# Fabstir/fabstir-vectordb

Hardware: AMD Instinct MI355X
Metric: k-NN queries/sec at recall@10>=0.95, 1Mx384 f32 (higher is better)
Workload: dtype f32

## Files before the change

fabstir-vectordb_amd/csrc/fvdb_hip.cpp:

```cpp
#include "fvdb_internal.h"

#include <unistd.h>

#include <algorithm>
#include <atomic>
#include <cmath>
#include <condition_variable>
#include <mutex>
#include <cstdio>
#include <cstdlib>
#include <cstring>
#include <map>
#include <new>
#include <string>
#include <vector>

#include "common.h"
#include "pool.h"
#include "kernels_misc.h"
#include "kernels_scan.h"
#include "kernels_wide.h"
#include "kernels_range.h"
#include "kernels_rank.h"
#include "kernels_curve.h"
#include "kernels_coarse.h"
#include "kernels_mfma.h"
#include "kernels_mfma_wg.h"
#include "kernels_util.h"
#include "kernels_maint.h"
#include "kernels_rows.h"

using namespace fvdb;


enum FbWord : uint32_t {
  FB_COARSE = 0,
  FB_SCAN = 1,
  FB_REASONS = 2,
  FB_OVERFLOW = 2,
  FB_REFINED = 6,
  FB_WORDS = 8,
};
constexpr size_t kFbBytes = FB_WORDS * 4;
constexpr size_t kFbAllBytes = 2 * kFbBytes;
constexpr uint32_t kFbReasonWords = 5;

enum StageEvent {
  EV_COARSE_BEGIN = 0,
  EV_COARSE_SCANNED,
  EV_COARSE_DONE,
  EV_SCAN_BEGIN,
  EV_SCAN_DONE,
  EV_FINE_DONE,
  EV_FILTER_BEGIN,
  EV_FILTER_DONE,
  EV_COUNT
};

enum ScalWord : uint32_t {
  SC_COARSE_ITEMS = 0,
  SC_COARSE_HEAD = 1,
  SC_FINE_ITEMS = 2,
  SC_FINE_HEAD = 3,
  SC_STATS = 4,
};
constexpr size_t kScalarsBytes = 64;

struct IvfScratch {
  std::mutex enq;
  bool pend_filter = false;
  bool pending_profile = false, pend_coarse = false, pend_fine = false, collecting = false;
  DBuf s_qnorm, s_A;
  DBuf s_qh, s_qn2, s_thr, s_tA, s_pa, s_surv, s_scnt, s_fail, s_mslots;
  DBuf s_sdist, s_probes2;
  DBuf s_q, s_cpart, s_probes, s_cnt, s_fill, s_eoff, s_ioff, s_entries;
  DBuf s_part, s_scalars, s_ceoff, s_cioff;
  DBuf s_wbase, s_arena;
  DBuf s_wgbase;
  DBuf s_gwords, s_group;
  DBuf s_rbase, s_rarena;
  DBuf s_qual;
  DBuf s_clive, s_cprobes, s_ckeys, s_cval;
  DBuf s_in, s_slots, s_ids, s_clusters, s_out_ids, s_out_dist, s_out_cnt, s_cdist;
  DBuf s_fslots, s_frows;
  DevEvent fetch_done;
  DevEvent sev[EV_COUNT];
  uint32_t* scalar(ScalWord w) const { return s_scalars.as<uint32_t>() + w; }
};

struct fvdb_ivf : IvfScratch {
  static constexpr uint32_t kSlots = 16;
  IvfScratch spare[kSlots - 1];
  static constexpr uint32_t kLeases = 8;
  IvfScratch lease_set[kLeases];
  fvdb_ctx* lease_ctx[kLeases] = {};
  uint32_t lease_busy = 0;
  std::mutex mu;
  std::condition_variable lease_cv;
  std::atomic<IvfScratch*> last_set{nullptr};
  std::atomic<fvdb_ctx*> last_ctx{nullptr};
  fvdb_ctx* ctx = nullptr;
  uint32_t d = 0, dpad = 0, d4 = 0, nlist = 0;
  bool trained = false;
  bool f16 = false;

  std::vector<float> h_centroids;
  DBuf d_centroids_rm;
  DBuf d_cent_pad;
  DBuf d_cnorm, d_cnmax;
  DBuf s_fallbacks;
  uint32_t* fb_word(FbWord w, bool masked = false) const { return s_fallbacks.as<uint32_t>() + (masked ? FB_WORDS : 0) + w; }
  int coarse_mode = 0;
  int scan_mode = 0;
  HBuf h_fb;
  uint64_t mfma_q = 0;
  uint64_t fb_seen = 0, q_seen = 0;
  uint32_t exact_batches_left = 0;
  uint32_t backoff_len = 0;
  uint64_t overflow_seen = 0, overflow_q = 0;
  uint32_t refine_batches_left = 0;
  DBuf d_mfma_stamps;
  int mfma_stamps_launch = 0;
  DBuf d_xmax;
  Pool cpool;
  DBuf c_off, c_blocks, c_glob;

  Pool pool;
  std::vector<std::vector<uint32_t>> list_blocks;
  std::vector<uint32_t> list_len;
  uint64_t total_rows = 0;
  uint64_t mutations = 0;
  uint32_t max_list_blocks = 0;
  bool table_dirty = true;
  DBuf t_off, t_blocks, t_glob, t_len;
  std::vector<uint32_t> glob_blocks_host;
  bool glob_set = false;

  DBuf m_seq, m_dest, m_ids;
  fvdb_ivf* m_src = nullptr;
  uint64_t m_rows = 0;
  bool m_assigned = false;
  bool m_store_job = false;
  fvdb_maintenance_info_t m_info{};

  fvdb_search_stats last_stats{};
  float stage_ms[8] = {0, 0, 0, 0, 0, 0, 0, 0};
  uint64_t stage_calls = 0;
};

namespace {
struct Env {
  fvdb_ctx* ctx;
  IvfScratch* S;
  const uint64_t* live = nullptr;
};
inline IvfScratch& slot_scratch(fvdb_ivf* ivf, uint32_t slot) { return slot == 0 ? *ivf : ivf->spare[slot - 1]; }
inline const uint64_t* live_words(const fvdb_ivf* ivf, const Env& E) { return E.live ? E.live : ivf->pool.valid(); }
inline PoolView list_pool(const fvdb_ivf* ivf, const Env& E) {
  PoolView v = ivf->pool.view();
  v.valid = live_words(ivf, E);
  return v;
}
}


namespace {

struct IvfKnobs {
  static int num(const char* name, int unset) { return getenv(name) ? atoi(getenv(name)) : unset; }
  static bool has(const char* name) { return getenv(name) != nullptr; }
  static int tiles(int m) { return m >= 4 ? 4 : (m >= 2 ? 2 : 1); }
  bool coarse_exact = has("FVDB_COARSE_EXACT");
  bool scan_exact = has("FVDB_SCAN_EXACT");
  uint32_t scan_wgs_per_cu = (uint32_t)num("FVDB_SCAN_WGS_PER_CU", 8);
  int segb = num("FVDB_SEGB", 0);
  bool no_shared_thr = has("FVDB_NO_SHARED_THR");
  int mfma_m = tiles(num("FVDB_MFMA_M", 2));
  int mfma_segb = num("FVDB_MFMA_SEGB", 0);
  uint32_t mfma_wgs_per_cu = (uint32_t)std::max(1, num("FVDB_MFMA_WGS_PER_CU", 2));
  bool mfma_groups_in_item = num("FVDB_MFMA_GROUPS_IN_ITEM", 0) != 0;
  bool mfma_wg = num("FVDB_MFMA_WG", 1) != 0;
  int mfma_wg_m = num("FVDB_MFMA_WG_M", 4) >= 4 ? 4 : 2;
  uint32_t mfma_wg_segb = (uint32_t)std::max(4, num("FVDB_MFMA_WG_SEGB", 16));
  uint32_t mfma_wg_per_cu = (uint32_t)std::max(1, num("FVDB_MFMA_WG_PER_CU", 2));
  int mfma_wg_tail_pct = num("FVDB_MFMA_WG_TAIL_PCT", 25);
  int mfma_wg_segb_tail = num("FVDB_MFMA_WG_SEGB_TAIL", 4);
  uint32_t mfma_cap_a = (uint32_t)std::max(1, num("FVDB_MFMA_CAP_A", 4));
  bool mfma_threshold_pass = has("FVDB_MFMA_THRESHOLD_PASS");
  uint32_t mfma_segb_a = (uint32_t)std::max(1, num("FVDB_MFMA_SEGB_A", 1));
  bool mfma_no_refine = has("FVDB_MFMA_NO_REFINE");
#ifdef FVDB_MFMA_STAMPS_BUILD
  int mfma_stamps = num("FVDB_MFMA_STAMPS", 0);
#endif
};
const IvfKnobs& ivf_knobs() {
  static const IvfKnobs knobs{};
  return knobs;
}

struct ScanLaunch {
  PoolView pool;
  const uint32_t* list_off;
  const uint32_t* list_blocks;
  uint32_t nlist;
  const uint32_t* entry_off;
  const uint32_t* item_off;
  const uint2* entries;
  const uint32_t* n_items;
  uint32_t* head;
  const float* queries;
  uint32_t dpad, segb, k, nprobe, maxsegs;
  uint2* part;
  uint32_t max_items = 0;
  bool f16 = false;
};

inline int kr_for(uint32_t k) { return k <= 64 ? 1 : (k <= 128 ? 2 : 4); }
inline uint32_t q_for(uint32_t k) { return k <= 64 ? 16u : (k <= 128 ? 8u : 4u); }

template <int Q, int KR, int ROLE, int ST>
void launch_scan_t(fvdb_ctx* ctx, const ScanLaunch& s) {
  uint32_t grid = (uint32_t)ctx->num_cus * ivf_knobs().scan_wgs_per_cu;
  if (s.max_items) grid = std::min(grid, std::max<uint32_t>(1u, (s.max_items + 3) / 4));
  hipLaunchKernelGGL((scan_topk_kernel<Q, KR, ROLE, ST>), dim3(grid), dim3(256), 0, ctx->stream, s.pool.data, s.pool.valid,
                     s.pool.d4, s.list_off, s.list_blocks, s.nlist, s.entry_off, s.item_off, (const u32x2*)s.entries,
                     s.n_items, s.head, s.queries, s.dpad, s.segb, s.k, s.nprobe, s.maxsegs, (u32x2*)s.part);
}

template <int ROLE, int ST>
void launch_scan_rs(fvdb_ctx* ctx, const ScanLaunch& s) {
  switch (kr_for(s.k)) {
    case 1: launch_scan_t<16, 1, ROLE, ST>(ctx, s); break;
    case 2: launch_scan_t<8, 2, ROLE, ST>(ctx, s); break;
    default: launch_scan_t<4, 4, ROLE, ST>(ctx, s); break;
  }
}
template <int ROLE>
void launch_scan_r(fvdb_ctx* ctx, const ScanLaunch& s) {
  if (s.f16) launch_scan_rs<ROLE, 1>(ctx, s); else launch_scan_rs<ROLE, 0>(ctx, s);
}
enum { ROLE_COARSE = 0, ROLE_LIST = 1, ROLE_ALL = 2 };
void launch_scan(fvdb_ctx* ctx, const ScanLaunch& s, int role) {
  if (role == ROLE_COARSE) launch_scan_r<ROLE_COARSE>(ctx, s);
  else if (role == ROLE_LIST) launch_scan_r<ROLE_LIST>(ctx, s);
  else launch_scan_r<ROLE_ALL>(ctx, s);
}

void launch_merge(fvdb_ctx* ctx, const MergeArgs& m) {
  const uint32_t grid = cdiv(m.B, 4);
  switch (kr_for(m.k)) {
    case 1: hipLaunchKernelGGL((merge_topk_kernel<1>), dim3(grid), dim3(256), 0, ctx->stream, m); break;
    case 2: hipLaunchKernelGGL((merge_topk_kernel<2>), dim3(grid), dim3(256), 0, ctx->stream, m); break;
    default: hipLaunchKernelGGL((merge_topk_kernel<4>), dim3(grid), dim3(256), 0, ctx->stream, m); break;
  }
}

int upload_table(fvdb_ivf* ivf) {
  fvdb_ctx* ctx = ivf->ctx;
  std::lock_guard<std::mutex> lk(ivf->mu);
  if (!ivf->table_dirty) return FVDB_OK;
  std::vector<uint32_t> off(ivf->nlist + 1, 0), blocks;
  std::vector<uint32_t> glob(ivf->nlist, 0);
  uint32_t mx = 0;
  for (uint32_t L = 0; L < ivf->nlist; ++L) {
    off[L] = (uint32_t)blocks.size();
    blocks.insert(blocks.end(), ivf->list_blocks[L].begin(), ivf->list_blocks[L].end());
    mx = std::max<uint32_t>(mx, (uint32_t)ivf->list_blocks[L].size());
    glob[L] = ivf->glob_set ? ivf->glob_blocks_host[L] : (uint32_t)ivf->list_blocks[L].size();
  }
  off[ivf->nlist] = (uint32_t)blocks.size();
  ivf->max_list_blocks = mx;
  HIPCHK(ctx, ivf->t_off.ensure(off.size() * 4));
  HIPCHK(ctx, ivf->t_blocks.ensure(std::max<size_t>(blocks.size(), 1) * 4));
  HIPCHK(ctx, ivf->t_glob.ensure(glob.size() * 4));
  HIPCHK(ctx, hipMemcpyAsync(ivf->t_off.p, off.data(), off.size() * 4, hipMemcpyHostToDevice, ctx->stream));
  if (!blocks.empty())
    HIPCHK(ctx, hipMemcpyAsync(ivf->t_blocks.p, blocks.data(), blocks.size() * 4, hipMemcpyHostToDevice, ctx->stream));
  HIPCHK(ctx, hipMemcpyAsync(ivf->t_glob.p, glob.data(), glob.size() * 4, hipMemcpyHostToDevice, ctx->stream));
  HIPCHK(ctx, ivf->t_len.ensure((size_t)ivf->nlist * 4));
  HIPCHK(ctx, hipMemcpyAsync(ivf->t_len.p, ivf->list_len.data(), (size_t)ivf->nlist * 4, hipMemcpyHostToDevice,
                             ctx->stream));
  HIPCHK(ctx, hipStreamSynchronize(ctx->stream));
  ivf->table_dirty = false;
  return FVDB_OK;
}

int padded_queries(fvdb_ivf* ivf, const Env& E, const float* q_dev, uint32_t B, const float** out) {
  fvdb_ctx* ctx = E.ctx;
  IvfScratch& S = *E.S;
  if (ivf->d == ivf->dpad) {
    *out = q_dev;
    return FVDB_OK;
  }
  HIPCHK(ctx, S.s_q.ensure((size_t)B * ivf->dpad * 4));
  const uint64_t tot = (uint64_t)B * ivf->dpad;
  hipLaunchKernelGGL(pad_rows_kernel, dim3(cdiv(tot, 256)), dim3(256), 0, ctx->stream, q_dev, ivf->d, ivf->dpad,
                     (uint64_t)B, S.s_q.as<float>());
  *out = S.s_q.as<float>();
  return FVDB_OK;
}

inline void mark(const fvdb_ivf* ivf, const Env& E, StageEvent e) {
  if (ivf->ctx->profiling) (void)hipEventRecord(E.S->sev[e], E.ctx->stream);
}

struct Batch {
  const float* qpad;
  const uint32_t* probes;
  uint32_t B, k, np;
  uint64_t* out_ids;
  float* out_dist;
  uint32_t* out_counts;
  uint64_t* out_keys;
  const float* given_thr = nullptr;
  bool glob_keys = false;
  const uint64_t* const* words = nullptr;
  const uint32_t* group = nullptr;
  const float* radius = nullptr;
  uint32_t* out_totals = nullptr;
};

inline ListTable list_table(const fvdb_ivf* ivf) {
  return ListTable{ivf->t_off.as<uint32_t>(), ivf->t_blocks.as<uint32_t>(), ivf->nlist};
}

MergeArgs merge_args(const PoolView& pool, const ListTable& lists, const uint32_t* glob_blocks, const DBuf& part,
                     uint32_t maxsegs, uint32_t segb, const Batch& b) {
  MergeArgs m{};
  m.pool = pool;
  m.lists = lists;
  m.probes = b.probes;
  m.glob_blocks = glob_blocks;
  m.part = part.as<uint2>();
  m.B = b.B;
  m.k = b.k;
  m.nprobe = b.np;
  m.maxsegs = maxsegs;
  m.segb = segb;
  m.out_ids = b.out_ids;
  m.out_dist = b.out_dist;
  m.out_counts = b.out_counts;
  m.out_keys = b.out_keys;
  return m;
}

constexpr uint64_t kRankArenaBytes = 256ull << 20;
int check_rank(fvdb_ctx* ctx, const fvdb_ivf* ivf, uint32_t np) {
  if (np > FVDB_MAX_K && ivf->nlist > kRankSortMaxLists)
    FAIL(ctx, FVDB_E_UNSUPPORTED, "nprobe above FVDB_MAX_K needs an index of at most 16384 lists");
  return FVDB_OK;
}

int run_coarse_rank(fvdb_ivf* ivf, const Env& E, const float* qpad, uint32_t B, uint32_t kc, uint32_t* out_probes,
                    float* out_dist) {
  fvdb_ctx* ctx = E.ctx;
  IvfScratch& S = *E.S;
  int rc = check_rank(ctx, ivf, kc);
  if (rc) return rc;
  const uint32_t cblocks = ivf->cpool.used_blocks, n = cblocks * 64;
  uint32_t P = 1;
  while (P < n) P <<= 1;
  const uint32_t lds = P * 8;
  const uint32_t threads = std::min<uint32_t>(kRankThreads, std::max<uint32_t>(64, P / 2));
  const uint32_t chunk = (uint32_t)std::min<uint64_t>(B, std::max<uint64_t>(1, kRankArenaBytes / ((uint64_t)n * 4)));
  HIPCHK(ctx, S.s_rarena.ensure((size_t)chunk * n * 4));
  HIPCHK(ctx, S.s_rbase.ensure((size_t)chunk * 2 * 4));
  HIPCHK(ctx, S.s_entries.ensure((size_t)chunk * 8));
  HIPCHK(ctx, S.s_ceoff.ensure(16));
  HIPCHK(ctx, S.s_cioff.ensure(16));
  HIPCHK(ctx, S.s_scalars.ensure(kScalarsBytes));
  HIPCHK(ctx, hipFuncSetAttribute((const void*)rank_sort_kernel, hipFuncAttributeMaxDynamicSharedMemorySize,
                                  (int)(kRankSortMaxLists * 8)));
  const ListTable clist{ivf->c_off.as<uint32_t>(), ivf->c_blocks.as<uint32_t>(), 1};
  const PoolView cpool = ivf->cpool.view();
  const uint32_t grid = (uint32_t)ctx->num_cus * ivf_knobs().scan_wgs_per_cu;
  mark(ivf, E, EV_COARSE_BEGIN);
  for (uint32_t o = 0; o < B; o += chunk) {
    const uint32_t b = std::min(chunk, B - o);
    hipLaunchKernelGGL(plan_all_kernel, dim3(cdiv(b, 256)), dim3(256), 0, ctx->stream, b, cblocks, 1u, 16u,
                       S.s_ceoff.as<uint32_t>(), S.s_cioff.as<uint32_t>(), S.s_entries.as<uint2>(),
                       S.scalar(SC_COARSE_ITEMS), S.scalar(SC_COARSE_HEAD));
    hipLaunchKernelGGL(rank_base_kernel, dim3(cdiv(b, 256)), dim3(256), 0, ctx->stream, b, cblocks, S.s_rbase.as<uint32_t>());
    const uint32_t items = cblocks * cdiv(b, 16);
    hipLaunchKernelGGL(wide_score_kernel<0>, dim3(std::min(grid, std::max<uint32_t>(1u, cdiv(items, 4)))), dim3(256), 0,
                       ctx->stream, cpool.data, cpool.valid, cpool.d4, clist.off, clist.blocks, 1u, S.s_ceoff.as<uint32_t>(),
                       S.s_cioff.as<uint32_t>(), (const u32x2*)S.s_entries.as<uint2>(), S.scalar(SC_COARSE_ITEMS),
                       S.scalar(SC_COARSE_HEAD), qpad + (size_t)o * ivf->dpad, ivf->dpad, 1u, 1u, S.s_rbase.as<uint32_t>(),
                       S.s_rarena.as<uint32_t>(), (uint64_t)n);
    if (o + b == B) mark(ivf, E, EV_COARSE_SCANNED);
    RankArgs r{};
    r.pool = cpool;
    r.lists = clist;
    r.arena = S.s_rarena.as<uint32_t>();
    r.n = n;
    r.P = P;
    r.np = kc;
    r.out_probes = out_probes + (size_t)o * kc;
    r.out_dist = out_dist ? out_dist + (size_t)o * kc : nullptr;
    hipLaunchKernelGGL(rank_sort_kernel, dim3(b), dim3(threads), lds, ctx->stream, r);
  }
  mark(ivf, E, EV_COARSE_DONE);
  HIPCHK(ctx, hipGetLastError());
  return FVDB_OK;
}

int run_coarse(fvdb_ivf* ivf, const Env& E, const float* qpad, uint32_t B, uint32_t kc, uint32_t* out_probes,
               float* out_dist) {
  fvdb_ctx* ctx = E.ctx;
  IvfScratch& S = *E.S;
  if (kc > FVDB_MAX_K) return run_coarse_rank(ivf, E, qpad, B, kc, out_probes, out_dist);
  if (ivf->coarse_mode == 0 && !ivf_knobs().coarse_exact && ivf->dpad % 16 == 0 && kc <= 48 && ivf->nlist >= 64 && B > 0 &&
      (uint64_t)B * ivf->nlist < (1ull << 31)) {
    const uint32_t nlist = ivf->nlist;
    const float* cpad = ivf->d == ivf->dpad ? ivf->d_centroids_rm.as<float>() : ivf->d_cent_pad.as<float>();
    HIPCHK(ctx, S.s_qnorm.ensure((size_t)B * 4));
    HIPCHK(ctx, S.s_A.ensure((size_t)B * nlist * 4));
    mark(ivf, E, EV_COARSE_BEGIN);
    hipLaunchKernelGGL(row_sqnorm_wave_kernel, dim3(cdiv(B, 4)), dim3(256), 0, ctx->stream, qpad, ivf->dpad, ivf->dpad, B,
                       S.s_qnorm.as<float>());
    const uint32_t waves = cdiv(B, 32) * cdiv(nlist, 64);
    hipLaunchKernelGGL(coarse_gemm_kernel, dim3(cdiv(waves, 4)), dim3(256), 0, ctx->stream, qpad, cpad,
                       S.s_qnorm.as<float>(), ivf->d_cnorm.as<float>(), B, nlist, ivf->dpad, S.s_A.as<float>());
    mark(ivf, E, EV_COARSE_SCANNED);
    hipLaunchKernelGGL(coarse_select_kernel, dim3(cdiv(B, 4)), dim3(256), 0, ctx->stream, S.s_A.as<float>(), qpad, cpad,
                       S.s_qnorm.as<float>(), ivf->d_cnmax.as<float>(), B, nlist, ivf->d, ivf->dpad, 64u, kc,
                       out_probes, out_dist, ivf->fb_word(FB_COARSE));
    mark(ivf, E, EV_COARSE_DONE);
    HIPCHK(ctx, hipGetLastError());
    return FVDB_OK;
  }
  const uint32_t cblocks = ivf->cpool.used_blocks;
  const uint32_t segb = 1, Q = q_for(kc);
  const uint32_t maxsegs = cblocks;
  HIPCHK(ctx, S.s_cpart.ensure((size_t)B * maxsegs * kc * 8));
  HIPCHK(ctx, S.s_entries.ensure((size_t)B * std::max<uint32_t>(kc, 1) * 8));
  HIPCHK(ctx, S.s_ceoff.ensure(16));
  HIPCHK(ctx, S.s_cioff.ensure(16));
  HIPCHK(ctx, S.s_scalars.ensure(kScalarsBytes));
  hipLaunchKernelGGL(plan_all_kernel, dim3(cdiv(std::max<uint32_t>(B, 1), 256)), dim3(256), 0, ctx->stream, B, cblocks,
                     segb, Q, S.s_ceoff.as<uint32_t>(), S.s_cioff.as<uint32_t>(), S.s_entries.as<uint2>(),
                     S.scalar(SC_COARSE_ITEMS), S.scalar(SC_COARSE_HEAD));
  const ListTable clist{ivf->c_off.as<uint32_t>(), ivf->c_blocks.as<uint32_t>(), 1};
  ScanLaunch s{ivf->cpool.view(), clist.off, clist.blocks, 1, S.s_ceoff.as<uint32_t>(), S.s_cioff.as<uint32_t>(),
               S.s_entries.as<uint2>(), S.scalar(SC_COARSE_ITEMS), S.scalar(SC_COARSE_HEAD), qpad, ivf->dpad, segb, kc, 1,
               maxsegs, S.s_cpart.as<uint2>(), cdiv(cblocks, segb) * cdiv(B, Q)};
  mark(ivf, E, EV_COARSE_BEGIN);
  launch_scan(ctx, s, ROLE_COARSE);
  mark(ivf, E, EV_COARSE_SCANNED);
  MergeArgs m = merge_args(ivf->cpool.view(), clist, ivf->c_glob.as<uint32_t>(), S.s_cpart, maxsegs, segb,
                           Batch{qpad, nullptr, B, kc, 1, nullptr, out_dist, nullptr, nullptr});
  m.out_probes = out_probes;
  launch_merge(ctx, m);
  mark(ivf, E, EV_COARSE_DONE);
  HIPCHK(ctx, hipGetLastError());
  return FVDB_OK;
}

uint32_t segb_for(uint32_t max_blocks, uint32_t B, uint32_t nprobe) {
  const uint64_t pairs = (uint64_t)B * nprobe;
  if (max_blocks >= 4096) return 16;
  if (pairs >= 4096) return 4;
  if (pairs >= 512) return 2;
  return 1;
}
uint32_t pick_segb(fvdb_ivf* ivf, uint32_t B, uint32_t nprobe) {
  const int forced = ivf_knobs().segb;
  return forced > 0 ? (uint32_t)forced : segb_for(ivf->max_list_blocks, B, nprobe);
}
uint64_t queries_per_gib(uint32_t max_blocks, uint32_t segb, uint32_t k, uint32_t np) {
  const uint64_t per_q = (uint64_t)np * std::max<uint32_t>(1, cdiv(max_blocks, segb)) * k * 8;
  return (1ull << 30) / std::max<uint64_t>(per_q, 1);
}

void launch_plan(fvdb_ivf* ivf, const Env& E, const uint32_t* probes, uint32_t n, uint32_t np, uint32_t segb, uint32_t Q,
                 unsigned long long* stats, uint32_t* rezero_cnt, uint32_t lsplit = 0xFFFFFFFFu, uint32_t segb_tail = 0) {
  fvdb_ctx* ctx = E.ctx;
  IvfScratch& S = *E.S;
  const uint32_t* list_off = ivf->t_off.as<uint32_t>();
  hipLaunchKernelGGL(plan_count_kernel, dim3(cdiv(n, 256)), dim3(256), 0, ctx->stream, probes, n, S.s_cnt.as<uint32_t>(),
                     list_off);
  hipLaunchKernelGGL(plan_scan_kernel, dim3(1), dim3(1024), 0, ctx->stream, S.s_cnt.as<uint32_t>(), list_off,
                     ivf->t_len.as<uint32_t>(), ivf->nlist, segb, Q, S.s_eoff.as<uint32_t>(), S.s_ioff.as<uint32_t>(),
                     S.s_fill.as<uint32_t>(), S.scalar(SC_FINE_ITEMS), S.scalar(SC_FINE_HEAD), stats, rezero_cnt, lsplit,
                     segb_tail);
  hipLaunchKernelGGL(plan_fill_kernel, dim3(cdiv(n, 256)), dim3(256), 0, ctx->stream, probes, n, np,
                     S.s_eoff.as<uint32_t>(), S.s_fill.as<uint32_t>(), S.s_entries.as<uint2>(), list_off);
}
inline unsigned long long* scan_stats(const IvfScratch& S) { return (unsigned long long*)S.scalar(SC_STATS); }

int plan_scratch(fvdb_ivf* ivf, const Env& E, uint32_t B, uint32_t np) {
  fvdb_ctx* ctx = E.ctx;
  IvfScratch& S = *E.S;
  const uint32_t nlist = ivf->nlist;
  HIPCHK(ctx, S.s_cnt.ensure((size_t)nlist * 4));
  HIPCHK(ctx, S.s_fill.ensure((size_t)nlist * 4));
  HIPCHK(ctx, S.s_eoff.ensure((size_t)(nlist + 1) * 4));
  HIPCHK(ctx, S.s_ioff.ensure((size_t)(nlist + 1) * 4));
  HIPCHK(ctx, S.s_entries.ensure((size_t)B * np * 8));
  return FVDB_OK;
}

int run_fine_exact(fvdb_ivf* ivf, const Env& E, const Batch& b, int role) {
  fvdb_ctx* ctx = E.ctx;
  IvfScratch& S = *E.S;
  const uint32_t nlist = ivf->nlist;
  const uint32_t segb = pick_segb(ivf, b.B, b.np), Q = q_for(b.k);
  const uint32_t maxsegs = std::max<uint32_t>(1, cdiv(ivf->max_list_blocks, segb));
  const uint64_t part_elems = (uint64_t)b.B * b.np * maxsegs * b.k;
  if (part_elems >= (1ull << 32)) FAIL(ctx, FVDB_E_UNSUPPORTED, "batch too large for one launch (sub-batch it)");
  int rc = plan_scratch(ivf, E, b.B, b.np);
  if (rc) return rc;
  HIPCHK(ctx, S.s_part.ensure((size_t)part_elems * 8));
  HIPCHK(ctx, S.s_scalars.ensure(kScalarsBytes));
  HIPCHK(ctx, hipMemsetAsync(S.s_cnt.p, 0, (size_t)nlist * 4, ctx->stream));
  launch_plan(ivf, E, b.probes, b.B * b.np, b.np, segb, Q, scan_stats(S), nullptr);
  mark(ivf, E, EV_SCAN_BEGIN);
  const ListTable lists = list_table(ivf);
  ScanLaunch s{list_pool(ivf, E), lists.off, lists.blocks, nlist, S.s_eoff.as<uint32_t>(), S.s_ioff.as<uint32_t>(),
               S.s_entries.as<uint2>(), S.scalar(SC_FINE_ITEMS), S.scalar(SC_FINE_HEAD), b.qpad, ivf->dpad, segb, b.k, b.np,
               maxsegs, S.s_part.as<uint2>()};
  s.f16 = ivf->f16;
  launch_scan(ctx, s, role);
  mark(ivf, E, EV_SCAN_DONE);
  launch_merge(ctx, merge_args(list_pool(ivf, E), lists, ivf->t_glob.as<uint32_t>(), S.s_part, maxsegs, segb, b));
  mark(ivf, E, EV_FINE_DONE);
  HIPCHK(ctx, hipGetLastError());
  return FVDB_OK;
}

constexpr uint32_t kMfmaSlack = 6;
constexpr uint32_t kMfmaCmax = 4096;

bool mfma_shape_ok(const fvdb_ivf* ivf, uint32_t B, uint32_t k, uint32_t np) {
  return ivf->dpad % 16 == 0 && k + kMfmaSlack <= 32 && np <= 256 && B >= 32 && B <= 16384;
}
inline bool half_rows(const fvdb_ivf* ivf) { return ivf->f16 || ivf->pool.half() != nullptr; }
inline int x_rounded(const fvdb_ivf* ivf) { return ivf->f16 ? 0 : (ivf->pool.half() ? 1 : 2); }

struct MfmaPlan {
  bool wg;
  int M;
  uint32_t Q, ka, cmax;
  uint32_t segb, segbA;
  uint32_t lsplit, segb_tail;
  uint32_t fsegb, fmaxsegs;
  uint64_t fpart;
  uint32_t grid, wg_grid, wg_lds;
  bool half_rows;
  int x_rounded;
};

int mfma_plan(fvdb_ivf* ivf, fvdb_ctx* ctx, const IvfKnobs& kn, uint32_t B, uint32_t k, uint32_t np, MfmaPlan* out) {
  MfmaPlan P{};
  P.half_rows = half_rows(ivf);
  P.x_rounded = x_rounded(ivf);
  int wgM = kn.mfma_wg_m;
  if (mfma_wg_lds_bytes(ivf->dpad, 16u * wgM) > 64u * 1024u) wgM = 2;
  P.wg = kn.mfma_wg && kn.mfma_m == 2 && P.half_rows && ivf->dpad % 128 == 0 &&
         mfma_wg_lds_bytes(ivf->dpad, 16u * wgM) <= 64u * 1024u;
  P.M = P.wg ? wgM : kn.mfma_m;
  P.Q = 16u * P.M;
  P.ka = k + kMfmaSlack;
  P.cmax = kMfmaCmax;
  P.segbA = kn.mfma_segb_a;
  P.segb = P.wg ? kn.mfma_wg_segb : (kn.mfma_segb > 0 ? (uint32_t)kn.mfma_segb : pick_segb(ivf, B, np));
  P.lsplit = 0xFFFFFFFFu;
  P.segb_tail = P.segb;
  if (P.wg && kn.mfma_wg_tail_pct > 0 && kn.mfma_wg_segb_tail > 0 && (uint32_t)kn.mfma_wg_segb_tail < P.segb) {
    P.lsplit = (uint32_t)((uint64_t)ivf->nlist * (uint32_t)(100 - std::min(kn.mfma_wg_tail_pct, 100)) / 100);
    P.segb_tail = (uint32_t)kn.mfma_wg_segb_tail;
  }
  P.fsegb = pick_segb(ivf, B, np);
  P.fmaxsegs = std::max<uint32_t>(1, cdiv(ivf->max_list_blocks, P.fsegb));
  P.fpart = (uint64_t)B * np * P.fmaxsegs * k;
  if (P.fpart >= (1ull << 32)) FAIL(ctx, FVDB_E_UNSUPPORTED, "batch too large for one launch (sub-batch it)");
  P.grid = (uint32_t)ctx->num_cus * kn.mfma_wgs_per_cu;
  P.wg_grid = (uint32_t)ctx->num_cus * kn.mfma_wg_per_cu;
// ... 2333 lines not shown
```

fabstir-vectordb_amd/csrc/kernels_coarse.h:

```cpp
#pragma once
#include "common.h"
#include "kernels_scan.h"
#include "score_rows.h"

#pragma clang fp contract(off)

namespace fvdb {

typedef float f32x16v __attribute__((ext_vector_type(16)));

__global__ void row_sqnorm_kernel(const float* __restrict__ x, uint32_t stride, uint32_t d, uint32_t n,
                                  float* __restrict__ norms) {
  const uint32_t i = blockIdx.x * blockDim.x + threadIdx.x;
  if (i >= n) return;
  const float* r = x + (size_t)i * stride;
  float s = 0.0f;
  for (uint32_t j = 0; j < d; ++j) s += r[j] * r[j];
  norms[i] = s;
}

__global__ __launch_bounds__(256) void row_sqnorm_wave_kernel(const float* __restrict__ x, uint32_t stride, uint32_t d,
                                                              uint32_t n, float* __restrict__ norms) {
  const int lane = threadIdx.x & 63;
  const uint32_t i = blockIdx.x * 4 + (threadIdx.x >> 6);
  if (i >= n) return;
  const float* r = x + (size_t)i * stride;
  float s = 0.0f;
  for (uint32_t j = lane; j < d; j += 64) s = __builtin_fmaf(r[j], r[j], s);
#pragma unroll
  for (int o = 32; o > 0; o >>= 1) s += __shfl_xor(s, o);
  if (lane == 0) norms[i] = s;
}

__global__ void max_f32_kernel(const float* __restrict__ v, uint32_t n, float* __restrict__ out) {
  if (blockIdx.x == 0 && threadIdx.x == 0) {
    float m = 0.0f;
    for (uint32_t i = 0; i < n; ++i) m = fmaxf(m, v[i]);
    *out = m;
  }
}

__global__ __launch_bounds__(256) void coarse_gemm_kernel(const float* __restrict__ q, const float* __restrict__ c,
                                                          const float* __restrict__ qn, const float* __restrict__ cn,
                                                          uint32_t B, uint32_t nlist, uint32_t dpad,
                                                          float* __restrict__ A ) {
  const int lane = threadIdx.x & 63;
  const uint32_t wave = blockIdx.x * 4 + (threadIdx.x >> 6);
  const uint32_t tiles_c = (nlist + 63) / 64;
  const uint32_t tb = wave / tiles_c, tc = wave - tb * tiles_c;
  if (tb * 32 >= B) return;
  const uint32_t i = lane & 31, h = lane >> 5;
  const uint32_t qrow = min(tb * 32 + i, B - 1);
  const uint32_t c0row = min(tc * 64 + i, nlist - 1), c1row = min(tc * 64 + 32 + i, nlist - 1);
  const float4* qp = (const float4*)(q + (size_t)qrow * dpad + 8 * h);
  const float4* c0p = (const float4*)(c + (size_t)c0row * dpad + 8 * h);
  const float4* c1p = (const float4*)(c + (size_t)c1row * dpad + 8 * h);
  f32x16v acc0 = {0}, acc1 = {0};
  for (uint32_t k0 = 0; k0 < dpad; k0 += 16) {
    const float4 qa = qp[k0 / 4], qb = qp[k0 / 4 + 1];
    const float4 a0 = c0p[k0 / 4], b0 = c0p[k0 / 4 + 1];
    const float4 a1 = c1p[k0 / 4], b1 = c1p[k0 / 4 + 1];
    const float qv[8] = {qa.x, qa.y, qa.z, qa.w, qb.x, qb.y, qb.z, qb.w};
    const float v0[8] = {a0.x, a0.y, a0.z, a0.w, b0.x, b0.y, b0.z, b0.w};
    const float v1[8] = {a1.x, a1.y, a1.z, a1.w, b1.x, b1.y, b1.z, b1.w};
#pragma unroll
    for (int m = 0; m < 8; ++m) {
      acc0 = __builtin_amdgcn_mfma_f32_32x32x2f32(qv[m], v0[m], acc0, 0, 0, 0);
      acc1 = __builtin_amdgcn_mfma_f32_32x32x2f32(qv[m], v1[m], acc1, 0, 0, 0);
    }
  }
  const uint32_t col0 = tc * 64 + i, col1 = col0 + 32;
  const float cn0 = col0 < nlist ? cn[col0] : 0.0f, cn1 = col1 < nlist ? cn[col1] : 0.0f;
#pragma unroll
  for (int r = 0; r < 16; ++r) {
    const uint32_t row = tb * 32 + (r & 3) + 8 * (r >> 2) + 4 * h;
    if (row < B) {
      const float qq = qn[row];
      if (col0 < nlist) A[(size_t)row * nlist + col0] = fmaxf(qq + cn0 - 2.0f * acc0[r], 0.0f);
      if (col1 < nlist) A[(size_t)row * nlist + col1] = fmaxf(qq + cn1 - 2.0f * acc1[r], 0.0f);
    }
  }
}

__device__ __forceinline__ float exact_centroid_dist(const float* __restrict__ q, const float* __restrict__ crow,
                                                     uint32_t dpad) {
  float acc = 0.0f;
  for (uint32_t j = 0; j < dpad; j += 4) {
    const float4 qv = *(const float4*)(q + j), cv = *(const float4*)(crow + j);
    float t;
    t = qv.x - cv.x; acc = acc + t * t;
    t = qv.y - cv.y; acc = acc + t * t;
    t = qv.z - cv.z; acc = acc + t * t;
    t = qv.w - cv.w; acc = acc + t * t;
  }
  return sqrtf(acc);
}

constexpr int kCoarseRegs = 16;

__global__ __launch_bounds__(256) void coarse_select_kernel(const float* __restrict__ A, const float* __restrict__ q,
                                                            const float* __restrict__ c ,
                                                            const float* __restrict__ qn,
                                                            const float* __restrict__ cn_max, uint32_t B,
                                                            uint32_t nlist, uint32_t d, uint32_t dpad, uint32_t C,
                                                            uint32_t kc, uint32_t* __restrict__ out_probes,
                                                            float* __restrict__ out_dist,
                                                            uint32_t* __restrict__ n_exact_fallbacks) {
  __shared__ __attribute__((aligned(16))) float s_tile[4][kScoreTileFloats];
  const int lane = threadIdx.x & 63;
  const uint32_t b = __builtin_amdgcn_readfirstlane(blockIdx.x * 4 + (threadIdx.x >> 6));
  if (b >= B) return;
  const float* arow = A + (size_t)b * nlist;
  const float* qrow = q + (size_t)b * dpad;
  WaveTopK<1> prop;
  prop.init();
  uint32_t th = kInf32, tl = kInf32;
  if (nlist <= 64u * kCoarseRegs && C <= 64 && C >= 1) {
    __shared__ uint32_t s_sel[4][128];
    uint32_t* sel = s_sel[threadIdx.x >> 6];
    uint32_t v[kCoarseRegs];
    uint32_t lo = kInf32, hi = 0;
#pragma unroll
    for (int r = 0; r < kCoarseRegs; ++r) {
      const uint32_t cc = (uint32_t)r * 64u + (uint32_t)lane;
      v[r] = cc < nlist ? __float_as_uint(arow[cc]) : kInf32;
      lo = min(lo, v[r]);
      if (cc < nlist) hi = max(hi, v[r]);
    }
#pragma unroll
    for (int o = 32; o > 0; o >>= 1) {
      lo = min(lo, (uint32_t)__shfl_xor(lo, o));
      hi = max(hi, (uint32_t)__shfl_xor(hi, o));
    }
    auto count_le = [&](uint32_t t) {
      uint32_t cn = 0;
#pragma unroll
      for (int r = 0; r < kCoarseRegs; ++r) cn += __popcll(__ballot(v[r] <= t));
      return cn;
    };
    const uint32_t want = min(C, nlist);
    uint32_t a = lo, b = hi;
    while (a < b) {
      const uint32_t mid = a + ((b - a) >> 1);
      if (count_le(mid) >= want) b = mid;
      else a = mid + 1;
    }
    const uint32_t t = a;
    uint32_t n_lt = 0;
#pragma unroll
    for (int r = 0; r < kCoarseRegs; ++r) n_lt += __popcll(__ballot(v[r] < t));
    uint32_t w_lt = 0, w_eq = n_lt;
#pragma unroll
    for (int r = 0; r < kCoarseRegs; ++r) {
      const uint32_t cc = (uint32_t)r * 64u + (uint32_t)lane;
      const uint64_t ml = __ballot(v[r] < t), me = __ballot(v[r] == t && cc < nlist);
      const uint64_t below = (1ull << lane) - 1ull;
      if (v[r] < t) {
        const uint32_t sl = w_lt + __popcll(ml & below);
        sel[2 * sl] = v[r];
        sel[2 * sl + 1] = cc;
      } else if (v[r] == t && cc < nlist) {
        const uint32_t sl = w_eq + __popcll(me & below);
        if (sl < want) {
          sel[2 * sl] = v[r];
          sel[2 * sl + 1] = cc;
        }
      }
      w_lt += __popcll(ml);
      w_eq += __popcll(me);
    }
    __builtin_amdgcn_fence(__ATOMIC_ACQ_REL, "wavefront");
    __builtin_amdgcn_wave_barrier();
    uint32_t shi = kInf32, slo = kInf32;
    if ((uint32_t)lane < want) {
      shi = sel[2 * lane];
      slo = sel[2 * lane + 1];
    }
    wave_sort64(shi, slo, lane);
    prop.hi[0] = shi;
    prop.lo[0] = slo;
    prop.kth(C, th, tl);
  } else
  for (uint32_t c0 = 0; c0 < nlist; c0 += 64) {
    const uint32_t cc = c0 + lane;
    uint32_t chi = kInf32, clo = cc;
    if (cc < nlist) chi = __float_as_uint(arow[cc]);
    if (c0 == 0) {
      uint32_t shi = chi, slo = cc < nlist ? cc : kInf32;
      wave_sort64(shi, slo, lane);
      prop.hi[0] = shi;
      prop.lo[0] = slo;
      prop.kth(C, th, tl);
    } else {
      offer<1>(prop, C, chi, clo, th, tl, lane);
    }
  }
  const bool all_in = C >= nlist;
  uint32_t ehi = kInf32, elo = kInf32;
  const bool cand = (uint32_t)lane < C && prop.hi[0] != kInf32;
  const uint32_t ncand = __popcll(__ballot(cand));
  const float dex = score_rows_wave(c, dpad, qrow, cand ? prop.lo[0] : 0u, ncand, s_tile[threadIdx.x >> 6], lane);
  if (cand) {
    ehi = __float_as_uint(dex);
    elo = prop.lo[0];
  }
  wave_sort64(ehi, elo, lane);
  bool proven = all_in;
  if (!all_in) {
    const float a_c = __uint_as_float(th);
    const float nq = sqrtf(qn[b]), ncm = sqrtf(cn_max[0]);
    const float eps = 1.01f * (float)(d + 4) * 5.9604645e-8f * (nq + ncm) * (nq + ncm);
    const float lower = sqrtf(fmaxf(a_c - 2.0f * eps, 0.0f)) * (1.0f - 4.8e-7f);
    const uint32_t kk = min(kc, C);
    const float d_k = __uint_as_float(rlane(ehi, kk - 1));
    proven = rlane(ehi, kk - 1) != kInf32 && d_k < lower;
  }
  if (!proven) {
    WaveTopK<1> ex;
    ex.init();
    uint32_t xh = kInf32, xl = kInf32;
    for (uint32_t c0 = 0; c0 < nlist; c0 += 64) {
      const uint32_t cc = c0 + lane;
      uint32_t chi = kInf32;
      if (cc < nlist) chi = __float_as_uint(exact_centroid_dist(qrow, c + (size_t)cc * dpad, dpad));
      if (c0 == 0) {
        uint32_t shi = chi, slo = cc < nlist ? cc : kInf32;
        wave_sort64(shi, slo, lane);
        ex.hi[0] = shi;
        ex.lo[0] = slo;
        ex.kth(kc, xh, xl);
      } else {
        offer<1>(ex, kc, chi, cc, xh, xl, lane);
      }
    }
    ehi = ex.hi[0];
    elo = ex.lo[0];
    if (lane == 0 && n_exact_fallbacks) atomicAdd(n_exact_fallbacks, 1u);
  }
  if ((uint32_t)lane < kc) {
    const bool have = ehi != kInf32;
    out_probes[(size_t)b * kc + lane] = have ? elo : kInf32;
    if (out_dist) out_dist[(size_t)b * kc + lane] = have ? __uint_as_float(ehi) : __uint_as_float(0x7F800000u);
  }
}

}
```

fabstir-vectordb_amd/csrc/score_rows.h:

```cpp
#pragma once
#include "common.h"
#include "row_types.h"

#pragma clang fp contract(off)

namespace fvdb {

#ifndef FVDB_FAST_ADD_UNROLL
#define FVDB_FAST_ADD_UNROLL 16
#endif
constexpr int kScoreAddUnroll = FVDB_FAST_ADD_UNROLL;
constexpr uint32_t kScoreStride = 132;
constexpr uint32_t kScoreTileFloats = 16 * kScoreStride;

#ifdef FVDB_GRAPH_STAMPS
#define SCORE_STAMP_PARAM , unsigned long long* t_acc = nullptr
#define SCORE_STAMP(var) const unsigned long long var = __builtin_amdgcn_s_memtime()
#define SCORE_STAMP_ADD(slot, a, b) \
  do {                              \
    if (t_acc) t_acc[slot] += (b) - (a); \
  } while (0)
#else
#define SCORE_STAMP_PARAM
#define SCORE_STAMP(var)
#define SCORE_STAMP_ADD(slot, a, b)
#endif

template <typename P, int RC, int NB>
__device__ __forceinline__ void score_products(const P (&x)[RC][NB], int c, const float2 q, float* tile, int lane) {
#pragma unroll
  for (int r = 0; r < RC; ++r) {
    const float2 xv = row_widen(x[r][c]);
    const float t0 = q.x - xv.x, t1 = q.y - xv.y;
    *(float2*)(tile + (uint32_t)r * kScoreStride + 2u * (uint32_t)lane) = make_float2(t0 * t0, t1 * t1);
  }
}

template <int RC>
__device__ __forceinline__ uint32_t score_lane_row(int lane) {
  return (uint32_t)lane < (uint32_t)RC ? (uint32_t)lane : (uint32_t)(RC - 1);
}

__device__ __forceinline__ void score_tile_publish() {
  __builtin_amdgcn_fence(__ATOMIC_RELEASE, "wavefront");
  __builtin_amdgcn_wave_barrier();
}
__device__ __forceinline__ float score_add_row(const float* tile, uint32_t lrow, float acc) {
  const float4* p = (const float4*)(tile + lrow * kScoreStride);
#pragma unroll kScoreAddUnroll
  for (int i = 0; i < 32; ++i) {
    const float4 v = p[i];
    acc = acc + v.x;
    acc = acc + v.y;
    acc = acc + v.z;
    acc = acc + v.w;
  }
  return acc;
}
__device__ __forceinline__ void score_tile_retire() {
  __builtin_amdgcn_fence(__ATOMIC_ACQ_REL, "wavefront");
  __builtin_amdgcn_wave_barrier();
}
__device__ __forceinline__ float score_fold(const float* tile, uint32_t lrow, float acc) {
  score_tile_publish();
  acc = score_add_row(tile, lrow, acc);
  score_tile_retire();
  return acc;
}

template <int NB, int RC, bool FULL, int TILES, typename RT>
__device__ __forceinline__ float score_fixed(const RT* __restrict__ rows, uint32_t dpad, const float2 (&q2)[NB], uint32_t pn,
                                             uint32_t cnt, float* stage, uint32_t tile_floats, int lane SCORE_STAMP_PARAM) {
  static_assert(TILES == 1 || TILES == 2, "one or two product tiles");
  SCORE_STAMP(ta);
  using P = typename RowVec<RT>::Pair;
  P x[RC][NB];
  const uint32_t last = cnt - 1;
#pragma unroll
  for (int r = 0; r < RC; ++r) {
    const uint32_t rr = (uint32_t)r < last ? (uint32_t)r : last;
    const uint32_t node = __builtin_amdgcn_readlane(pn, rr);
    const RT* row = rows + (size_t)node * dpad;
#pragma unroll
    for (int c = 0; c < NB; ++c) {
      const uint32_t j = (uint32_t)c * 128u + 2u * (uint32_t)lane;
      if (FULL) x[r][c] = *(const P*)(row + j);
      else x[r][c] = j < dpad ? *(const P*)(row + j) : RowVec<RT>::zero_pair();
    }
  }
  SCORE_STAMP(tb);
  SCORE_STAMP_ADD(8, ta, tb);
  const uint32_t lrow = score_lane_row<RC>(lane);
  score_products(x, 0, q2[0], stage, lane);
  score_tile_publish();
  SCORE_STAMP(tc1);
  SCORE_STAMP_ADD(9, tb, tc1);
  float acc = 0.0f;
#pragma unroll
  for (int c = 0; c < NB; ++c) {
    const float* cur = TILES == 2 ? stage + (uint32_t)(c & 1) * tile_floats : stage;
    if (TILES == 2 && c + 1 < NB) score_products(x, c + 1, q2[c + 1], stage + (uint32_t)((c + 1) & 1) * tile_floats, lane);
    acc = score_add_row(cur, lrow, acc);
    score_tile_retire();
    if (TILES == 1 && c + 1 < NB) {
      score_products(x, c + 1, q2[c + 1], stage, lane);
      score_tile_publish();
    }
  }
  SCORE_STAMP(tc2);
  SCORE_STAMP_ADD(11, tc1, tc2);
  return sqrtf(acc);
}

template <int RC, typename RT>
__device__ __forceinline__ float score_rows_stream(const RT* __restrict__ rows, uint32_t dpad, const float* __restrict__ q, uint32_t pn,
                                                   uint32_t base, uint32_t cnt, float* tile, int lane) {
  const uint32_t nb = (dpad + 127) >> 7;
  using P = typename RowVec<RT>::Pair;
  const RT* rp[RC];
  const uint32_t last = cnt - 1;
#pragma unroll
  for (int r = 0; r < RC; ++r) {
    const uint32_t rr = (uint32_t)r < last ? (uint32_t)r : last;
    rp[r] = rows + (size_t)__builtin_amdgcn_readlane(pn, base + rr) * dpad;
  }
  const uint32_t j0 = 2u * (uint32_t)lane;
  auto load = [&](uint32_t c, P (&x)[RC][1], float2& qv) {
    const uint32_t j = c * 128u + j0;
    const bool in = j < dpad;
    qv = in ? *(const float2*)(q + j) : make_float2(0.0f, 0.0f);
#pragma unroll
    for (int r = 0; r < RC; ++r) x[r][0] = in ? *(const P*)(rp[r] + j) : RowVec<RT>::zero_pair();
  };
  const uint32_t lrow = score_lane_row<RC>(lane);
  float acc = 0.0f;
  auto fold = [&](const P (&x)[RC][1], const float2 qv) {
    score_products(x, 0, qv, tile, lane);
    acc = score_fold(tile, lrow, acc);
  };
  P xa[RC][1], xb[RC][1];
  float2 qa, qb;
  load(0, xa, qa);
  for (uint32_t c = 0; c < nb; c += 2) {
    if (c + 1 < nb) load(c + 1, xb, qb);
    fold(xa, qa);
    if (c + 1 < nb) {
      if (c + 2 < nb) load(c + 2, xa, qa);
      fold(xb, qb);
    }
  }
  return sqrtf(acc);
}

template <typename RT>
__device__ __forceinline__ float score_rows_upto16(const RT* __restrict__ rows, uint32_t dpad, const float* __restrict__ q, uint32_t pn,
                                                   uint32_t base, uint32_t cnt, float* tile, int lane) {
  if (cnt > 8) return score_rows_stream<16>(rows, dpad, q, pn, base, cnt, tile, lane);
  if (cnt > 4) return score_rows_stream<8>(rows, dpad, q, pn, base, cnt, tile, lane);
  return score_rows_stream<4>(rows, dpad, q, pn, base, cnt, tile, lane);
}

template <typename RT>
__device__ __forceinline__ float score_rows_wave(const RT* __restrict__ rows, uint32_t dpad, const float* __restrict__ q, uint32_t pn,
                                                 uint32_t n, float* tile, int lane) {
  float out = 0.0f;
  for (uint32_t base = 0; base < n; base += 16) {
    const uint32_t cnt = min(16u, n - base);
    const float d = score_rows_upto16(rows, dpad, q, pn, base, cnt, tile, lane);
    const float mine = __shfl(d, (int)((uint32_t)lane - base) & 63);
    if ((uint32_t)lane >= base && (uint32_t)lane < base + cnt) out = mine;
  }
  return out;
}

}
```

Before: 1.924 million.

## Tile coarse GEMM through LDS and widen coarse-select exact rescoring

Adds an LDS-tiled, double-buffered MFMA coarse GEMM kernel (64 queries by 128 centroids per block) with register prefetch of upcoming chunks. It replaces the per-wave GEMM by default so that query and centroid loads are shared across waves instead of reloaded by each one. The coarse select kernel also drops to 2 waves per block and rescores candidate centroids with a new wide scoring routine. That routine processes 64 rows in 32-float slabs, spreading rows across lane groups to improve load parallelism. The changes add sync overhead per chunk and more LDS per block, and the summation order in rescoring changes.

```diff
diff --git a/fabstir-vectordb_amd/csrc/fvdb_hip.cpp b/fabstir-vectordb_amd/csrc/fvdb_hip.cpp
--- a/fabstir-vectordb_amd/csrc/fvdb_hip.cpp
+++ b/fabstir-vectordb_amd/csrc/fvdb_hip.cpp
@@ -171,6 +171,7 @@
   static bool has(const char* name) { return getenv(name) != nullptr; }
   static int tiles(int m) { return m >= 4 ? 4 : (m >= 2 ? 2 : 1); }
   bool coarse_exact = has("FVDB_COARSE_EXACT");
+  bool coarse_gemm_tiled = num("FVDB_COARSE_GEMM", 1) != 0;
   bool scan_exact = has("FVDB_SCAN_EXACT");
   uint32_t scan_wgs_per_cu = (uint32_t)num("FVDB_SCAN_WGS_PER_CU", 8);
   int segb = num("FVDB_SEGB", 0);
@@ -418,11 +419,16 @@
     mark(ivf, E, EV_COARSE_BEGIN);
     hipLaunchKernelGGL(row_sqnorm_wave_kernel, dim3(cdiv(B, 4)), dim3(256), 0, ctx->stream, qpad, ivf->dpad, ivf->dpad, B,
                        S.s_qnorm.as<float>());
-    const uint32_t waves = cdiv(B, 32) * cdiv(nlist, 64);
-    hipLaunchKernelGGL(coarse_gemm_kernel, dim3(cdiv(waves, 4)), dim3(256), 0, ctx->stream, qpad, cpad,
-                       S.s_qnorm.as<float>(), ivf->d_cnorm.as<float>(), B, nlist, ivf->dpad, S.s_A.as<float>());
+    if (ivf_knobs().coarse_gemm_tiled) {
+      hipLaunchKernelGGL(coarse_gemm_tiled_kernel, dim3(cdiv(B, kCgTileQ) * cdiv(nlist, kCgTileC)), dim3(256), 0, ctx->stream,
+                         qpad, cpad, S.s_qnorm.as<float>(), ivf->d_cnorm.as<float>(), B, nlist, ivf->dpad, S.s_A.as<float>());
+    } else {
+      const uint32_t waves = cdiv(B, 32) * cdiv(nlist, 64);
+      hipLaunchKernelGGL(coarse_gemm_kernel, dim3(cdiv(waves, 4)), dim3(256), 0, ctx->stream, qpad, cpad,
+                         S.s_qnorm.as<float>(), ivf->d_cnorm.as<float>(), B, nlist, ivf->dpad, S.s_A.as<float>());
+    }
     mark(ivf, E, EV_COARSE_SCANNED);
-    hipLaunchKernelGGL(coarse_select_kernel, dim3(cdiv(B, 4)), dim3(256), 0, ctx->stream, S.s_A.as<float>(), qpad, cpad,
+    hipLaunchKernelGGL(coarse_select_kernel, dim3(cdiv(B, kCoarseSelWaves)), dim3(64 * kCoarseSelWaves), 0, ctx->stream, S.s_A.as<float>(), qpad, cpad,
                        S.s_qnorm.as<float>(), ivf->d_cnmax.as<float>(), B, nlist, ivf->d, ivf->dpad, 64u, kc,
                        out_probes, out_dist, ivf->fb_word(FB_COARSE));
     mark(ivf, E, EV_COARSE_DONE);
diff --git a/fabstir-vectordb_amd/csrc/kernels_coarse.h b/fabstir-vectordb_amd/csrc/kernels_coarse.h
--- a/fabstir-vectordb_amd/csrc/kernels_coarse.h
+++ b/fabstir-vectordb_amd/csrc/kernels_coarse.h
@@ -82,6 +82,86 @@
   }
 }
 
+constexpr uint32_t kCgTileQ = 64, kCgTileC = 128, kCgChunk = 8, kCgStride = 12;
+constexpr int kCgAhead = 4;
+
+__global__ __launch_bounds__(256) void coarse_gemm_tiled_kernel(const float* __restrict__ q, const float* __restrict__ c,
+                                                                const float* __restrict__ qn, const float* __restrict__ cn,
+                                                                uint32_t B, uint32_t nlist, uint32_t dpad,
+                                                                float* __restrict__ A ) {
+  __shared__ __attribute__((aligned(16))) float s_q[2][kCgTileQ * kCgStride];
+  __shared__ __attribute__((aligned(16))) float s_c[2][kCgTileC * kCgStride];
+  const uint32_t t = threadIdx.x, lane = t & 63, w = __builtin_amdgcn_readfirstlane(t >> 6);
+  const uint32_t tiles_c = (nlist + kCgTileC - 1) / kCgTileC;
+  const uint32_t tq = blockIdx.x / tiles_c, tc = blockIdx.x - tq * tiles_c;
+  const uint32_t q0 = tq * kCgTileQ, c0 = tc * kCgTileC;
+  const uint32_t srow = t >> 1, shalf = t & 1;
+  const bool carries_q = w < 2;
+  const float4* gc = (const float4*)(c + (size_t)min(c0 + srow, nlist - 1) * dpad) + shalf;
+  const float4* gq = (const float4*)(q + (size_t)min(q0 + (srow & (kCgTileQ - 1)), B - 1) * dpad) + shalf;
+  const uint32_t soff = srow * kCgStride + 4 * shalf;
+  const uint32_t nch = dpad / kCgChunk;
+  float4 rc[kCgAhead], rq[kCgAhead];
+#pragma unroll
+  for (int s = 0; s < kCgAhead; ++s) {
+    rc[s] = rq[s] = make_float4(0.0f, 0.0f, 0.0f, 0.0f);
+    if ((uint32_t)s < nch) {
+      rc[s] = gc[2 * s];
+      if (carries_q) rq[s] = gq[2 * s];
+    }
+  }
+  *(float4*)(s_c[0] + soff) = rc[0];
+  if (carries_q) *(float4*)(s_q[0] + soff) = rq[0];
+  if ((uint32_t)kCgAhead < nch) {
+    rc[0] = gc[2 * kCgAhead];
+    if (carries_q) rq[0] = gq[2 * kCgAhead];
+  }
+  __syncthreads();
+  const uint32_t i = lane & 31, h = lane >> 5;
+  const uint32_t fq = ((w & 1) * 32 + i) * kCgStride + 4 * h, fc = ((w >> 1) * 64 + i) * kCgStride + 4 * h;
+  f32x16v acc0 = {0}, acc1 = {0};
+  for (uint32_t k0 = 0; k0 < nch; k0 += kCgAhead) {
+#pragma unroll
+    for (int s = 0; s < kCgAhead; ++s) {
+      const uint32_t k = k0 + (uint32_t)s;
+      if (k < nch) {
+        const uint32_t buf = (uint32_t)s & 1;
+        const float4 a = *(const float4*)(s_q[buf] + fq);
+        const float4 b0 = *(const float4*)(s_c[buf] + fc), b1 = *(const float4*)(s_c[buf] + fc + 32 * kCgStride);
+        acc0 = __builtin_amdgcn_mfma_f32_32x32x2f32(a.x, b0.x, acc0, 0, 0, 0);
+        acc1 = __builtin_amdgcn_mfma_f32_32x32x2f32(a.x, b1.x, acc1, 0, 0, 0);
+        acc0 = __builtin_amdgcn_mfma_f32_32x32x2f32(a.y, b0.y, acc0, 0, 0, 0);
+        acc1 = __builtin_amdgcn_mfma_f32_32x32x2f32(a.y, b1.y, acc1, 0, 0, 0);
+        acc0 = __builtin_amdgcn_mfma_f32_32x32x2f32(a.z, b0.z, acc0, 0, 0, 0);
+        acc1 = __builtin_amdgcn_mfma_f32_32x32x2f32(a.z, b1.z, acc1, 0, 0, 0);
+        acc0 = __builtin_amdgcn_mfma_f32_32x32x2f32(a.w, b0.w, acc0, 0, 0, 0);
+        acc1 = __builtin_amdgcn_mfma_f32_32x32x2f32(a.w, b1.w, acc1, 0, 0, 0);
+        const int sn = (s + 1) % kCgAhead;
+        if (k + 1 < nch) {
+          *(float4*)(s_c[buf ^ 1] + soff) = rc[sn];
+          if (carries_q) *(float4*)(s_q[buf ^ 1] + soff) = rq[sn];
+          if (k + 1 + kCgAhead < nch) {
+            rc[sn] = gc[2 * (k + 1 + kCgAhead)];
+            if (carries_q) rq[sn] = gq[2 * (k + 1 + kCgAhead)];
+          }
+        }
+        __syncthreads();
+      }
+    }
+  }
+  const uint32_t col0 = c0 + (w >> 1) * 64 + i, col1 = col0 + 32;
+  const float cn0 = col0 < nlist ? cn[col0] : 0.0f, cn1 = col1 < nlist ? cn[col1] : 0.0f;
+#pragma unroll
+  for (int r = 0; r < 16; ++r) {
+    const uint32_t row = q0 + (w & 1) * 32 + (r & 3) + 8 * (r >> 2) + 4 * h;
+    if (row < B) {
+      const float qq = qn[row];
+      if (col0 < nlist) A[(size_t)row * nlist + col0] = fmaxf(qq + cn0 - 2.0f * acc0[r], 0.0f);
+      if (col1 < nlist) A[(size_t)row * nlist + col1] = fmaxf(qq + cn1 - 2.0f * acc1[r], 0.0f);
+    }
+  }
+}
+
 __device__ __forceinline__ float exact_centroid_dist(const float* __restrict__ q, const float* __restrict__ crow,
                                                      uint32_t dpad) {
   float acc = 0.0f;
@@ -98,7 +178,8 @@
 
 constexpr int kCoarseRegs = 16;
 
-__global__ __launch_bounds__(256) void coarse_select_kernel(const float* __restrict__ A, const float* __restrict__ q,
+constexpr uint32_t kCoarseSelWaves = 2;
+__global__ __launch_bounds__(64 * kCoarseSelWaves) void coarse_select_kernel(const float* __restrict__ A, const float* __restrict__ q,
                                                             const float* __restrict__ c ,
                                                             const float* __restrict__ qn,
                                                             const float* __restrict__ cn_max, uint32_t B,
@@ -106,9 +187,9 @@
                                                             uint32_t kc, uint32_t* __restrict__ out_probes,
                                                             float* __restrict__ out_dist,
                                                             uint32_t* __restrict__ n_exact_fallbacks) {
-  __shared__ __attribute__((aligned(16))) float s_tile[4][kScoreTileFloats];
+  __shared__ __attribute__((aligned(16))) float s_tile[kCoarseSelWaves][kWideTileFloats];
   const int lane = threadIdx.x & 63;
-  const uint32_t b = __builtin_amdgcn_readfirstlane(blockIdx.x * 4 + (threadIdx.x >> 6));
+  const uint32_t b = __builtin_amdgcn_readfirstlane(blockIdx.x * kCoarseSelWaves + (threadIdx.x >> 6));
   if (b >= B) return;
   const float* arow = A + (size_t)b * nlist;
   const float* qrow = q + (size_t)b * dpad;
@@ -116,7 +197,7 @@
   prop.init();
   uint32_t th = kInf32, tl = kInf32;
   if (nlist <= 64u * kCoarseRegs && C <= 64 && C >= 1) {
-    __shared__ uint32_t s_sel[4][128];
+    __shared__ uint32_t s_sel[kCoarseSelWaves][128];
     uint32_t* sel = s_sel[threadIdx.x >> 6];
     uint32_t v[kCoarseRegs];
     uint32_t lo = kInf32, hi = 0;
@@ -199,7 +280,7 @@
   uint32_t ehi = kInf32, elo = kInf32;
   const bool cand = (uint32_t)lane < C && prop.hi[0] != kInf32;
   const uint32_t ncand = __popcll(__ballot(cand));
-  const float dex = score_rows_wave(c, dpad, qrow, cand ? prop.lo[0] : 0u, ncand, s_tile[threadIdx.x >> 6], lane);
+  const float dex = score_rows_wide(c, dpad, qrow, cand ? prop.lo[0] : 0u, ncand, s_tile[threadIdx.x >> 6], lane);
   if (cand) {
     ehi = __float_as_uint(dex);
     elo = prop.lo[0];
diff --git a/fabstir-vectordb_amd/csrc/score_rows.h b/fabstir-vectordb_amd/csrc/score_rows.h
--- a/fabstir-vectordb_amd/csrc/score_rows.h
+++ b/fabstir-vectordb_amd/csrc/score_rows.h
@@ -45,10 +45,12 @@
   __builtin_amdgcn_fence(__ATOMIC_RELEASE, "wavefront");
   __builtin_amdgcn_wave_barrier();
 }
+template <uint32_t STRIDE = kScoreStride, int N4 = 32>
 __device__ __forceinline__ float score_add_row(const float* tile, uint32_t lrow, float acc) {
-  const float4* p = (const float4*)(tile + lrow * kScoreStride);
-#pragma unroll kScoreAddUnroll
-  for (int i = 0; i < 32; ++i) {
+  const float4* p = (const float4*)(tile + lrow * STRIDE);
+  constexpr int kUnroll = N4 < kScoreAddUnroll ? N4 : kScoreAddUnroll;
+#pragma unroll kUnroll
+  for (int i = 0; i < N4; ++i) {
     const float4 v = p[i];
     acc = acc + v.x;
     acc = acc + v.y;
@@ -173,4 +175,50 @@
   return out;
 }
 
-}
+constexpr uint32_t kWideSlab = 32;
+constexpr uint32_t kWideStride = kWideSlab + 4;
+constexpr uint32_t kWideTileFloats = 64 * kWideStride;
+constexpr int kWideLoads = 16;
+
+template <typename RT>
+__device__ __forceinline__ float score_rows_wide(const RT* __restrict__ rows, uint32_t dpad, const float* __restrict__ q, uint32_t pn,
+                                                 uint32_t n, float* tile, int lane) {
+  using P = typename RowVec<RT>::Pair;
+  const uint32_t sub = (uint32_t)lane >> 4, pj = 2u * ((uint32_t)lane & 15u);
+  const uint32_t last = n - 1;
+  uint32_t node[kWideLoads];
+#pragma unroll
+  for (int m = 0; m < kWideLoads; ++m) {
+    const uint32_t r = min(4u * (uint32_t)m + sub, last);
+    node[m] = __shfl(pn, (int)r);
+  }
+  const uint32_t ns = (dpad + kWideSlab - 1) / kWideSlab;
+  auto load = [&](uint32_t s, P (&x)[kWideLoads], float2& qv) {
+    const uint32_t j = s * kWideSlab;
+    const bool in = j + pj < dpad;
+    qv = in ? *(const float2*)(q + j + pj) : make_float2(0.0f, 0.0f);
+#pragma unroll
+    for (int m = 0; m < kWideLoads; ++m)
+      x[m] = in ? *(const P*)(rows + (size_t)node[m] * dpad + (j + pj)) : RowVec<RT>::zero_pair();
+  };
+  const uint32_t lrow = min((uint32_t)lane, last);
+  float acc = 0.0f;
+  P x[kWideLoads];
+  float2 qv;
+  load(0, x, qv);
+  for (uint32_t s = 0; s < ns; ++s) {
+#pragma unroll
+    for (int m = 0; m < kWideLoads; ++m) {
+      const float2 xv = row_widen(x[m]);
+      const float t0 = qv.x - xv.x, t1 = qv.y - xv.y;
+      *(float2*)(tile + (4u * (uint32_t)m + sub) * kWideStride + pj) = make_float2(t0 * t0, t1 * t1);
+    }
+    if (s + 1 < ns) load(s + 1, x, qv);
+    score_tile_publish();
+    acc = score_add_row<kWideStride, (int)kWideSlab / 4>(tile, lrow, acc);
+    score_tile_retire();
+  }
+  return sqrtf(acc);
+}
+
+}
```

Result: no change. 1.911 million, median of 2 (-0.7%).
